# AndreasKarg/raytracer-weekend

Measured on AMD Instinct MI355X. Metric: Mrays/sec at 1920x1080, 512 spp, 50 bounces; 1/2/4/8-GPU scaling, higher is better.
Workload: dtype f32; 1 GPU; Random-spheres scene, 1920x1080, 512 spp, 1xMI355X (configs[1]); scene=jumpy-balls, width=1920, height=1080, spp=512, max_depth=50, rays_per_frame=3103484398, tiles=32400, launches_per_frame=1, parallelism=tiles1

## Files before the change

raytracer-weekend_amd/csrc/rtw_dev_trace.hpp:

```cpp
#pragma once
#include "rtw_dev_hit.hpp"

namespace rtw {
namespace dev {

struct TraceState {
  Best b;
  int32_t node;
  int32_t pend;
  int32_t sp;
  bool on;
};

template <int AXIS, bool FAST>
__device__ __forceinline__ void rect_list_test(const Ray& lr, V3 y, float4 q0, float k, uint32_t pi, float& bt,
                                               int32_t& bp) {
  const float o_k = AXIS == 0 ? lr.o.z : (AXIS == 1 ? lr.o.y : lr.o.x);
  const float d_k = AXIS == 0 ? lr.d.z : (AXIS == 1 ? lr.d.y : lr.d.x);
  const float y_k = AXIS == 0 ? y.z : (AXIS == 1 ? y.y : y.x);
  const float o_a = AXIS == 2 ? lr.o.y : lr.o.x, d_a = AXIS == 2 ? lr.d.y : lr.d.x;
  const float o_b = AXIS == 0 ? lr.o.y : lr.o.z, d_b = AXIS == 0 ? lr.d.y : lr.d.z;
  const float num = k - o_k;
  bool acc;
  if constexpr (FAST) {
    const float t = div_by_recip(num, d_k, y_k);
    const float x = o_a + t * d_a;
    const float yy = o_b + t * d_b;
    const float m1 = __builtin_amdgcn_fmed3f(t, TMIN, bt), m2 = __builtin_amdgcn_fmed3f(x, q0.x, q0.y);
    const float m3 = __builtin_amdgcn_fmed3f(yy, q0.z, q0.w);
    acc = fmaxf(fmaxf(fabsf(m1 - t), fabsf(m2 - x)), fabsf(m3 - yy)) == 0.0f;
    bt = acc ? t : bt;
    bp = acc ? (int32_t)pi : bp;
  } else {
    const float t = num / d_k;
    const float x = o_a + t * d_a;
    const float yy = o_b + t * d_b;
    const bool out = (x < q0.x) | (x > q0.y) | (yy < q0.z) | (yy > q0.w);
    acc = !(t < TMIN) & !(t > bt) & !out;
    const bool tnan = t != t;
    bt = acc ? (tnan ? INFINITY : t) : bt;
    bp = acc ? ((int32_t)pi | (tnan ? RECT_NAN_HIT : 0)) : bp;
  }
}

template <bool COUNT, int AXIS, bool FAST>
__device__ __forceinline__ void rect_list_run(const DevScene& S, uint32_t first, uint32_t count, const Ray& lr, V3 y,
                                              float& bt, int32_t& bp, uint32_t* cnt) {
  typedef uint32_t u8v __attribute__((ext_vector_type(8)));
  const __attribute__((address_space(4))) u8v* P = (const __attribute__((address_space(4))) u8v*)(S.prims + first);
  auto one = [&](const u8v& rec, uint32_t k) {
    const float4 q0 = make_float4(__uint_as_float(rec[0]), __uint_as_float(rec[1]), __uint_as_float(rec[2]),
                                  __uint_as_float(rec[3]));
    rect_list_test<AXIS, FAST>(lr, y, q0, __uint_as_float(rec[4]), first + k, bt, bp);
    if (COUNT) { cnt[1]++; cnt[2 + PT_RECT_XY + AXIS]++; simd_tick(cnt, 10, 11); }
  };
  uint32_t k = 0;
  const __attribute__((address_space(4))) u8v* Pk = P;
  for (; k + 1u < count; k += 2u, Pk += 4) {
    const u8v r0 = Pk[0], r1 = Pk[2];
    one(r0, k);
    one(r1, k + 1u);
  }
  if (k < count) {
    const u8v rl = Pk[0];
    one(rl, k);
  }
}

template <bool COUNT, bool FAST>
__device__ __forceinline__ void rect_box6_run(const DevScene& S, uint32_t first, const Ray& lr, V3 y, float& bt,
                                              int32_t& bp, uint32_t* cnt) {
  rect_list_run<COUNT, 0, FAST>(S, first, 2u, lr, y, bt, bp, cnt);
  rect_list_run<COUNT, 1, FAST>(S, first + 2u, 2u, lr, y, bt, bp, cnt);
  rect_list_run<COUNT, 2, FAST>(S, first + 4u, 2u, lr, y, bt, bp, cnt);
}

template <bool COUNT>
__device__ __forceinline__ void trace_rect_list(const DevScene& S, const Ray& r, Best& best, uint32_t* cnt) {
  float bt = INFINITY;
  int32_t bp = -1;
  uint32_t cur = 0xFFFFFFFFu;
  Ray lr = r;
  V3 y = mk(0.f, 0.f, 0.f);
  bool fast = false;
  for (uint32_t g = 0; g < S.n_lgroups; ++g) {
    const uint4 G = uload(reinterpret_cast<const uint4*>(S.lgroups + g));
    if (G.z != cur) {
      cur = G.z;
      lr = r;
      if (cur) {
        const DevInst* I = S.insts + cur;
        const uint32_t n = uload(&I->nops);
        const float4 op0 = uload(reinterpret_cast<const float4*>(I->op[0]));
        const float4 op1 = uload(reinterpret_cast<const float4*>(I->op[1]));
        auto apply = [&](const float4& op) {
          if (op_is(op.x, IO_TRANSLATE)) {
            lr.o = sub(lr.o, mk(op.y, op.z, op.w));
          } else {
            const float sn = op.y, c = op.z;
            lr.o = mk(c * lr.o.x - sn * lr.o.z, lr.o.y, sn * lr.o.x + c * lr.o.z);
            lr.d = mk(c * lr.d.x - sn * lr.d.z, lr.d.y, sn * lr.d.x + c * lr.d.z);
          }
        };
        if (n >= 1u) apply(op0);
        if (n >= 2u) apply(op1);
        for (uint32_t k = 2; k < n; ++k) apply(uload(reinterpret_cast<const float4*>(I->op[k])));
      }
      y = mk(rcp_rn_fast(lr.d.x), rcp_rn_fast(lr.d.y), rcp_rn_fast(lr.d.z));
      const float dmin = fminf(fminf(fabsf(lr.d.x), fabsf(lr.d.y)), fabsf(lr.d.z));
      const float dsum = (fabsf(lr.d.x) + fabsf(lr.d.y)) + fabsf(lr.d.z);
      const float osum = (fabsf(lr.o.x) + fabsf(lr.o.y)) + fabsf(lr.o.z);
      const bool ok = (dmin >= 0x1p-60f) & (dsum <= 0x1p60f) & (osum < 0x1p62f);
      fast = S.rect_fast && __ballot(!ok) == 0;
    }
    if (fast) {
      if (G.w == GK_BOX6) rect_box6_run<COUNT, true>(S, G.x, lr, y, bt, bp, cnt);
      else if (G.w == PT_RECT_XY) rect_list_run<COUNT, 0, true>(S, G.x, G.y, lr, y, bt, bp, cnt);
      else if (G.w == PT_RECT_XZ) rect_list_run<COUNT, 1, true>(S, G.x, G.y, lr, y, bt, bp, cnt);
      else rect_list_run<COUNT, 2, true>(S, G.x, G.y, lr, y, bt, bp, cnt);
    } else {
      if (G.w == GK_BOX6) rect_box6_run<COUNT, false>(S, G.x, lr, y, bt, bp, cnt);
      else if (G.w == PT_RECT_XY) rect_list_run<COUNT, 0, false>(S, G.x, G.y, lr, y, bt, bp, cnt);
      else if (G.w == PT_RECT_XZ) rect_list_run<COUNT, 1, false>(S, G.x, G.y, lr, y, bt, bp, cnt);
      else rect_list_run<COUNT, 2, false>(S, G.x, G.y, lr, y, bt, bp, cnt);
    }
  }
  const bool nan_hit = bp >= 0 && (bp & RECT_NAN_HIT) != 0;
  best.t = nan_hit ? __builtin_nanf("") : bt;
  best.prim = nan_hit ? (bp & ~RECT_NAN_HIT) : bp;
}

__device__ __forceinline__ const DevFar* far_record(const DevScene& S) {
  const char* p = reinterpret_cast<const char*>(S.prims);
  asm volatile("" : "+s"(p));
  return reinterpret_cast<const DevFar*>(p - DEVFAR_BACK);
}
__device__ __forceinline__ float cull_inv(float d) {
  const float dd = fabsf(d) > 1e-20f ? d : copysignf(1e-20f, d);
  return __builtin_amdgcn_rcpf(dd);
}
__device__ __forceinline__ float cull_tmax(float t) { return __builtin_fmaf(t, 1.0e-5f, t) + 1.0e-5f; }
template <bool COUNT, uint32_t FEAT, int STACK, int BLK, bool C16, int NCAP>
__device__ void trace_far(const DevScene& S, const Ray& r, Best& b, float delta, uint16_t* stk16, int32_t* stk,
                          uint32_t* cnt, uint64_t seg, uint32_t* err, const float4* lnodes) {
  const DevFar* const FR = far_record(S);
  const char* const NB = NCAP > 0 ? reinterpret_cast<const char*>(lnodes)
                                  : reinterpret_cast<const char*>(S.prims) - uload(&FR->nodes_back);
  const uint32_t n_bvh = uload(&FR->n_bvh);
  const V3 inv = mk(cull_inv(r.d.x), cull_inv(r.d.y), cull_inv(r.d.z));
  const V3 ood = mk(r.o.x * inv.x, r.o.y * inv.y, r.o.z * inv.z);
  const V3 bn = mk(-ood.x - delta * fabsf(inv.x), -ood.y - delta * fabsf(inv.y), -ood.z - delta * fabsf(inv.z));
  const V3 bf = mk(-ood.x + delta * fabsf(inv.x), -ood.y + delta * fabsf(inv.y), -ood.z + delta * fabsf(inv.z));
  const uint32_t nx = inv.x < 0.f ? 16u : 0u, ny = (inv.y < 0.f ? 16u : 0u) + 32u, nz = (inv.z < 0.f ? 16u : 0u) + 64u;
  const uint32_t fx = nx ^ 16u, fy = ny ^ 16u, fz = nz ^ 16u;
  int32_t node = 0, sp = 0;
  bool over = false;
  for (uint32_t guard = 0;; ++guard) {
    if (node < 0) {
      if (sp == 0) break;
      --sp;
      node = C16 ? (int32_t)stk16[sp * BLK] : stk[sp * BLK];
    }
    if (guard >= (1u << 20)) {
      *err = 1u;
      b.prim = -2;
      return;
    }
    if (COUNT) cnt[0]++;
    const uint32_t nb = (uint32_t)node << 7;
    const float4 qnx = *reinterpret_cast<const float4*>(NB + (nb + nx)), qfx = *reinterpret_cast<const float4*>(NB + (nb + fx));
    const float4 qny = *reinterpret_cast<const float4*>(NB + (nb + ny)), qfy = *reinterpret_cast<const float4*>(NB + (nb + fy));
    const float4 qnz = *reinterpret_cast<const float4*>(NB + (nb + nz)), qfz = *reinterpret_cast<const float4*>(NB + (nb + fz));
    const uint4 cw = *reinterpret_cast<const uint4*>(NB + (nb + (C16 ? 112u : 96u)));
    const float tmax_c = cull_tmax(b.t);
    const float NX[4] = {qnx.x, qnx.y, qnx.z, qnx.w}, FX[4] = {qfx.x, qfx.y, qfx.z, qfx.w};
    const float NY[4] = {qny.x, qny.y, qny.z, qny.w}, FY[4] = {qfy.x, qfy.y, qfy.z, qfy.w};
    const float NZ[4] = {qnz.x, qnz.y, qnz.z, qnz.w}, FZ[4] = {qfz.x, qfz.y, qfz.z, qfz.w};
    const uint32_t W[4] = {cw.x, cw.y, cw.z, cw.w};
    uint32_t hits = 0;
    float tnear = INFINITY;
    int kn = -1;
#pragma unroll
    for (int k = 0; k < 4; ++k) {
      const float tn = fmaxf(fmaxf(fmaxf(__builtin_fmaf(NX[k], inv.x, bn.x), __builtin_fmaf(NY[k], inv.y, bn.y)),
                                   __builtin_fmaf(NZ[k], inv.z, bn.z)), 0.0f);
      const float tf = fminf(fminf(fminf(__builtin_fmaf(FX[k], inv.x, bf.x), __builtin_fmaf(FY[k], inv.y, bf.y)),
                                   __builtin_fmaf(FZ[k], inv.z, bf.z)), tmax_c);
      const bool h = W[k] != 0u && tn <= tf;
      hits |= h ? 1u << k : 0u;
      const bool inner = C16 ? (W[k] & 0x8000u) == 0u : (int32_t)W[k] >= 0;
      const bool nearer = h && inner && tn < tnear;
      tnear = nearer ? tn : tnear;
      kn = nearer ? k : kn;
    }
    node = kn < 0 ? -1 : (int32_t)(kn == 0 ? W[0] : (kn == 1 ? W[1] : (kn == 2 ? W[2] : W[3])));
    hits &= kn < 0 ? hits : ~(1u << kn);
    while (hits) {
      const int k = __builtin_ctz(hits);
      hits &= hits - 1u;
      const uint32_t w = k == 0 ? W[0] : (k == 1 ? W[1] : (k == 2 ? W[2] : W[3]));
      if (C16 ? (w & 0x8000u) != 0u : (int32_t)w < 0) {
        const uint32_t v = C16 ? w & 0xFFFFu : ~w;
        const uint32_t first = C16 ? (v >> 2) & 0x1FFFu : v >> 3, n = C16 ? (v & 3u) + 1u : v & 7u;
        for (uint32_t q = 0; q < n; ++q) test_prim<COUNT, FEAT>(S, first + q, r, b, cnt, seg);
      } else if (sp < STACK) {
        if constexpr (C16) stk16[sp * BLK] = (uint16_t)w;
        else stk[sp * BLK] = (int32_t)w;
        ++sp;
      } else {
        over = true;
      }
    }
  }
  if (over)
    for (uint32_t pi = 0; pi < n_bvh; ++pi) test_prim<COUNT, FEAT>(S, pi, r, b, cnt, seg);
}

constexpr bool far_kernel_feat(uint32_t feat) {
  return !(feat & F_LIST) && (feat & (F_SPHERE | F_MSPHERE | F_MEDIUM)) && feat != F_MESHES;
}
template <bool COUNT, uint32_t FEAT, int STACK = 1, int BLK = BLOCK, bool C16 = false, int NCAP = 0, bool RING = false>
__device__ __forceinline__ void trace_begin(const DevScene& S, const Ray& r, TraceState& ts, uint32_t* cnt,
                                            uint64_t seg, uint16_t* stk16 = nullptr, int32_t* stk = nullptr,
                                            uint32_t* err = nullptr, const float4* lnodes = nullptr,
                                            int32_t start = -3) {
  ts.b = Best{INFINITY, 0u, -1, 0.0f, 0.0f};
  const bool decided = RING && start != -3;
  constexpr bool RECT_LIST = (FEAT & F_LIST) && (FEAT & F_RECT) && !(FEAT & (F_SPHERE | F_MSPHERE | F_TRI | F_MEDIUM));
  if constexpr (RECT_LIST) {
    trace_rect_list<COUNT>(S, r, ts.b, cnt);
  } else if (FEAT & F_INST) {
    uint32_t cur = 0;
    Ray lr = r;
    const uint32_t a0 = S.n_prims - S.n_always;
    for (uint32_t k = 0; k < S.n_always; ++k) {
      const uint32_t pi = a0 + k;
      const uint32_t inst = uload(&S.prims[pi].type_inst) >> 8;
      if (inst != cur) {
        lr = inst ? to_local<true>(S.insts + inst, r) : r;
        cur = inst;
      }
      test_prim<COUNT, FEAT, true, true>(S, pi, lr, ts.b, cnt, seg);
    }
  } else if constexpr (RING) {
    const SphRcp rq = sph_rcp(r);
    const uint32_t n = decided ? (start >= 0 ? 1u : 0u) : S.n_always;
    for (uint32_t k = 0; __any(k < n); ++k) {
      if (k < n) {
        const uint32_t pi = decided ? (uint32_t)start : uload(S.always + k);
        test_prim<COUNT, FEAT, false, false>(S, pi, r, ts.b, cnt, seg, &rq);
      }
    }
  } else {
    constexpr bool SPH_ONLY = (FEAT & (F_RECT | F_TRI | F_MEDIUM | F_INST)) == 0 && (FEAT & (F_SPHERE | F_MSPHERE));
    SphRcp rq;
    if constexpr (SPH_ONLY) rq = sph_rcp(r);
    for (uint32_t k = 0; k < S.n_always; ++k)
      test_prim<COUNT, FEAT, false, true>(S, uload(S.always + k), r, ts.b, cnt, seg, SPH_ONLY ? &rq : nullptr);
  }
  if constexpr ((FEAT & F_LIST) && !RECT_LIST) {
    const bool nan_hit = ts.b.prim >= 0 && (ts.b.prim & RECT_NAN_HIT) != 0;
    ts.b.t = nan_hit ? __builtin_nanf("") : ts.b.t;
    ts.b.prim = nan_hit ? (ts.b.prim & ~RECT_NAN_HIT) : ts.b.prim;
  }
  bool walk = true;
#if defined(RTW_DIAG_FAR)
  constexpr int DF = RTW_DIAG_FAR;
#else
  constexpr int DF = 0;
#endif
  constexpr bool FAR = DF != 1 && far_kernel_feat(FEAT);
  if constexpr (FAR) {
    if (S.far_check) {
      const float4* const FR = reinterpret_cast<const float4*>(far_record(S));
      const float4 mid = uload(FR), half = uload(FR + 1);
      const float tx = fabsf(r.o.x - mid.x) + half.x;
      const float ty = fabsf(r.o.y - mid.y) + half.y;
      const float tz = fabsf(r.o.z - mid.z) + half.z;
      const float D2 = tx * tx + ty * ty + tz * tz;
      const bool far = D2 > mid.w && !decided;
      if (__any(far)) {
        bool need = false;
        float delta = 0.0f;
        if (far && DF != 2) {
          const float4 lo = uload(FR + 2), hi = uload(FR + 3), e = uload(FR + 4);
          const float D = __builtin_amdgcn_sqrtf(D2) * 1.000001f;
          delta = fminf(half.w * D2 + lo.w, hi.w * D + e.x) + (e.y * D + e.z);
          const float ix = __builtin_amdgcn_rcpf(r.d.x), iy = __builtin_amdgcn_rcpf(r.d.y), iz = __builtin_amdgcn_rcpf(r.d.z);
          const float ox = r.o.x - mid.x, oy = r.o.y - mid.y, oz = r.o.z - mid.z;
          const float hx = half.x + delta, hy = half.y + delta, hz = half.z + delta;
          const float ax = (-hx - ox) * ix, bx = (hx - ox) * ix, ay = (-hy - oy) * iy, by = (hy - oy) * iy;
          const float az = (-hz - oz) * iz, bz = (hz - oz) * iz;
          const float tn = fmaxf(fmaxf(fminf(ax, bx), fminf(ay, by)), fmaxf(fminf(az, bz), 0.0f));
          const float tf = fminf(fminf(fmaxf(ax, bx), fmaxf(ay, by)),
                                 fminf(fmaxf(az, bz), cull_tmax(ts.b.t)));
          need = tn <= tf;
        }
        walk = !far;
        if (DF == 5) asm volatile("" ::"v"((uint32_t)need));
        if (DF != 3 && DF != 5 && __builtin_expect(__any(need), 0))
          if (need) trace_far<COUNT, FEAT, STACK, BLK, C16, NCAP>(S, r, ts.b, delta, stk16, stk, cnt, seg, err, lnodes);
      }
    }
  }
  int32_t root = S.n_nodes ? 0 : -1;
  if constexpr ((FEAT & F_TRI) != 0) {
    root = __builtin_amdgcn_readfirstlane(root);
    asm volatile("" : "+s"(root));
  } else {
    asm volatile("" : "+v"(root));
  }
  ts.node = (walk && !decided) ? root : -1;
  ts.pend = 0;
  ts.sp = 0;
  ts.on = true;
}

#ifndef RTW_MESH_ROOT
#define RTW_MESH_ROOT 5
#endif
#ifndef REGEN_RING
#define REGEN_RING 2
#endif
#ifndef REGEN_RING_LDSN
#define REGEN_RING_LDSN 8
#endif
typedef _Float16 half2_t __attribute__((ext_vector_type(2)));
__device__ __forceinline__ half2_t as_h2(uint32_t u) { return __builtin_bit_cast(half2_t, u); }

template <bool COUNT, int STACK, bool SPILL, uint32_t FEAT, int BLK, int NCAP, bool HN = false, bool S16 = false>
__device__ void trace_run(const DevScene& S, const Ray& r, TraceState& ts, int32_t* stk, int32_t* spill,
                          uint32_t spill_lanes, uint32_t* cnt, uint32_t quota, uint32_t leaf_thr, uint64_t seg,
                          uint32_t* err, uint64_t* tph, const float4* lnodes, uint16_t* stk16) {
  constexpr bool K16 = NCAP > 0;
  constexpr bool CODES = K16 || HN || S16;
  constexpr bool SPH_ONLY = (FEAT & (F_RECT | F_TRI | F_MEDIUM | F_INST)) == 0 && (FEAT & (F_SPHERE | F_MSPHERE));
  SphRcp rq;
  if constexpr (SPH_ONLY) rq = sph_rcp(r);
  Ray tri_ray = r;
  if constexpr ((FEAT & F_TRI) != 0) {
    if (S.bvh_tri && (FEAT & F_INST) && S.tri_inst) {
      if (S.tri_inst == S.uni_inst) tri_ray.o = sub(r.o, mk(S.uni_off[0], S.uni_off[1], S.uni_off[2]));
      else tri_ray = to_local<true>(S.insts + S.tri_inst, r);
    }
  }
  uint64_t tm = COUNT ? __builtin_amdgcn_s_memtime() : 0;
  if constexpr (NCAP == 0) __builtin_amdgcn_s_setprio(2);
  auto tick = [&](int k) {
    if (COUNT) {
      const uint64_t t = __builtin_amdgcn_s_memtime();
      tph[k] += t - tm;
      tm = t;
    }
  };
  const V3 inv = mk(cull_inv(r.d.x), cull_inv(r.d.y), cull_inv(r.d.z));
  const V3 ood = mk(r.o.x * inv.x, r.o.y * inv.y, r.o.z * inv.z);
  const uint32_t nx = inv.x < 0.f ? 16u : 0u, ny = (inv.y < 0.f ? 16u : 0u) + 32u, nz = (inv.z < 0.f ? 16u : 0u) + 64u;
  const uint32_t fx = nx ^ 16u, fy = ny ^ 16u, fz = nz ^ 16u;
  const char* const NB = NCAP > 0 ? reinterpret_cast<const char*>(lnodes)
                                  : (HN ? reinterpret_cast<const char*>(S.hnodes) : reinterpret_cast<const char*>(S.nodes));
  constexpr bool ROOT = HN && S16 && NCAP == 0 && RTW_MESH_ROOT > 0;
  constexpr int32_t NROOT = RTW_MESH_ROOT;
#pragma unroll
  for (int lv = 0; lv < (ROOT ? (NROOT > 1 ? 2 : 1) : 0); ++lv) {
    if (__any(ts.node >= 0 && ts.node < NROOT)) {
      if (ts.node >= 0 && ts.node < NROOT) {
        const char* const TB = reinterpret_cast<const char*>(lnodes) + (uint32_t)ts.node * 112u;
        const uint4 px = *reinterpret_cast<const uint4*>(TB + nx);
        const uint4 py = *reinterpret_cast<const uint4*>(TB + ny);
        const uint4 pz = *reinterpret_cast<const uint4*>(TB + nz);
        const uint4 cq = *reinterpret_cast<const uint4*>(TB + 96u);
        const half2_t oxy = as_h2(cq.z), oz = as_h2(cq.w);
        const V3 bs = mk(__builtin_fmaf((float)oxy.x, inv.x, -ood.x), __builtin_fmaf((float)oxy.y, inv.y, -ood.y),
                         __builtin_fmaf((float)oz.x, inv.z, -ood.z));
        const uint32_t PQ[3][4] = {{px.x, px.y, px.z, px.w}, {py.x, py.y, py.z, py.w}, {pz.x, pz.y, pz.z, pz.w}};
        float NA[3][4], FA[3][4];
#pragma unroll
        for (int q = 0; q < 3; ++q) {
          const half2_t n01 = as_h2(PQ[q][0]), n23 = as_h2(PQ[q][1]), f01 = as_h2(PQ[q][2]), f23 = as_h2(PQ[q][3]);
          NA[q][0] = (float)n01.x; NA[q][1] = (float)n01.y; NA[q][2] = (float)n23.x; NA[q][3] = (float)n23.y;
          FA[q][0] = (float)f01.x; FA[q][1] = (float)f01.y; FA[q][2] = (float)f23.x; FA[q][3] = (float)f23.y;
        }
        const int32_t CW[4] = {(int32_t)(int16_t)(cq.x & 0xFFFFu), (int32_t)cq.x >> 16, (int32_t)(int16_t)(cq.y & 0xFFFFu),
                               (int32_t)cq.y >> 16};
        if (COUNT) {
          cnt[0]++;
          cnt[14] += (CW[0] != 0) + (CW[1] != 0) + (CW[2] != 0) + (CW[3] != 0);
        }
        const float tmax_c = cull_tmax(ts.b.t);
        int32_t next = -1, bk = -1;
        float best = INFINITY;
        bool hit[4];
#pragma unroll
        for (int k = 0; k < 4; ++k) {
          const float a0 = __builtin_fmaf(NA[0][k], inv.x, bs.x), b0 = __builtin_fmaf(NA[1][k], inv.y, bs.y);
          const float c0 = __builtin_fmaf(NA[2][k], inv.z, bs.z);
          const float d0 = __builtin_fmaf(FA[0][k], inv.x, bs.x), e0 = __builtin_fmaf(FA[1][k], inv.y, bs.y);
          const float f0 = __builtin_fmaf(FA[2][k], inv.z, bs.z);
          const float tn = fmaxf(fmaxf(fmaxf(a0, b0), c0), 0.0f);
          hit[k] = tn <= fminf(fminf(fminf(d0, e0), f0), tmax_c);
          const bool in = hit[k] & (CW[k] >= 0) & (tn < best);
          best = in ? tn : best;
          bk = in ? k : bk;
          next = in ? CW[k] : next;
        }
        int32_t pend = ts.pend, sp = ts.sp;
#pragma unroll
        for (int k = 0; k < 4; ++k) {
          const bool leaf_take = hit[k] & (CW[k] < 0) & (pend == 0);
          pend = leaf_take ? CW[k] : pend;
          const bool pk = hit[k] & (k != bk) & !leaf_take;
          stk16[sp * BLK] = (uint16_t)CW[k];
          sp += pk ? 1 : 0;
        }
        ts.pend = pend;
        ts.sp = sp;
        ts.node = next;
      }
    }
  }
  constexpr uint32_t GUARD = 1u << 20;
  uint32_t guard = 0;
  for (; guard < GUARD; ++guard) {
    uint32_t g2 = 0;
    for (; g2 < GUARD; ++g2) {
      if constexpr (K16) {
        const bool can = ts.node < 0 && ts.sp > 0;
        const int32_t top = can ? (int32_t)stk16[(ts.sp - 1) * BLK] : 0;
        const bool leaf = (top & 0x8000) != 0;
        const bool popn = can && !leaf;
        const bool popl = can && leaf && ts.pend == 0;
        ts.node = popn ? top : ts.node;
        ts.pend = popl ? top : ts.pend;
        ts.sp -= (popn || popl) ? 1 : 0;
      } else {
        const bool can = ts.node < 0 && ts.sp > 0;
        int32_t top = 0;
        if (can) {
          const int32_t i = ts.sp - 1;
          if constexpr (S16) {
            top = (int32_t)(int16_t)stk16[i * BLK];
          } else {
            top = stk[(SPILL ? min(i, STACK) : i) * BLK];
            if (SPILL && i >= STACK) top = spill[(size_t)(i - STACK) * spill_lanes];
          }
        }
        const bool popn = can && top >= 0;
        const bool popl = can && top < 0 && ts.pend == 0;
        ts.node = popn ? top : ts.node;
        ts.pend = popl ? top : ts.pend;
        ts.sp -= (popn || popl) ? 1 : 0;
      }
#ifdef RTW_LANE_DIAG
      if (COUNT) {
        const uint64_t bd = __ballot(ts.node >= 0), bp = __ballot(ts.node < 0 && ts.pend != 0);
        const uint64_t bn = __ballot(ts.node < 0 && ts.pend == 0 && ts.sp == 0);
        tph[3] += 64;
        tph[4] += (uint64_t)__popcll(bd);
        tph[5] += (uint64_t)__popcll(bp);
        tph[6] += (uint64_t)__popcll(bn);
      }
#endif
      if (!__any(ts.node >= 0 && ts.pend == 0)) break;
      if ((uint32_t)__popcll(__ballot(ts.node < 0 && ts.pend != 0)) >= leaf_thr) break;
#ifdef RTW_UNI_DIAG
      if (COUNT) {
        const uint64_t vis = __ballot(ts.node >= 0);
        const int src = (int)__ffsll((long long)vis) - 1;
        const int32_t n0 = __shfl(ts.node, src, 64);
        const uint32_t oct = nx | ny | nz, o0 = (uint32_t)__shfl((int)oct, src, 64);
        const bool un = __ballot(ts.node >= 0 && ts.node != n0) == 0;
        const bool uo = __ballot(ts.node >= 0 && (ts.node != n0 || oct != o0)) == 0;
        tph[3] += 1;
        tph[4] += uo ? 1 : 0;
        tph[5] += un ? 1 : 0;
        tph[6] += (uint64_t)__popcll(vis);
      }
#endif
      if (ts.node >= 0) {
        float NX[4], FX[4], NY[4], FY[4], NZ[4], FZ[4];
        int32_t CW[4];
        V3 bs;
        if constexpr (HN) {
          const uint32_t nb = (uint32_t)ts.node * 112u;
          const uint4 px = *reinterpret_cast<const uint4*>(NB + (nb + nx));
          const uint4 py = *reinterpret_cast<const uint4*>(NB + (nb + ny));
          const uint4 pz = *reinterpret_cast<const uint4*>(NB + (nb + nz));
          const uint4 cq = *reinterpret_cast<const uint4*>(NB + (nb + 96u));
          const half2_t oxy = as_h2(cq.z), oz = as_h2(cq.w);
          bs = mk(__builtin_fmaf((float)oxy.x, inv.x, -ood.x), __builtin_fmaf((float)oxy.y, inv.y, -ood.y),
                  __builtin_fmaf((float)oz.x, inv.z, -ood.z));
          const uint32_t P[3][4] = {{px.x, px.y, px.z, px.w}, {py.x, py.y, py.z, py.w}, {pz.x, pz.y, pz.z, pz.w}};
          float* const NA[3] = {NX, NY, NZ};
          float* const FA[3] = {FX, FY, FZ};
#pragma unroll
          for (int a = 0; a < 3; ++a) {
            const half2_t n01 = as_h2(P[a][0]), n23 = as_h2(P[a][1]), f01 = as_h2(P[a][2]), f23 = as_h2(P[a][3]);
            NA[a][0] = (float)n01.x; NA[a][1] = (float)n01.y; NA[a][2] = (float)n23.x; NA[a][3] = (float)n23.y;
            FA[a][0] = (float)f01.x; FA[a][1] = (float)f01.y; FA[a][2] = (float)f23.x; FA[a][3] = (float)f23.y;
          }
          if constexpr (K16) {
            CW[0] = (int32_t)(cq.x & 0xFFFFu); CW[1] = (int32_t)(cq.x >> 16);
            CW[2] = (int32_t)(cq.y & 0xFFFFu); CW[3] = (int32_t)(cq.y >> 16);
          } else {
            CW[0] = (int32_t)(int16_t)(cq.x & 0xFFFFu); CW[1] = (int32_t)cq.x >> 16;
            CW[2] = (int32_t)(int16_t)(cq.y & 0xFFFFu); CW[3] = (int32_t)cq.y >> 16;
          }
        } else {
          const uint32_t nb = (uint32_t)ts.node << 7;
          constexpr uint32_t CWO = (K16 || S16) ? 112u : 96u;
          const float4 qnx = *reinterpret_cast<const float4*>(NB + (nb + nx));
          const float4 qfx = *reinterpret_cast<const float4*>(NB + (nb + fx));
          const float4 qny = *reinterpret_cast<const float4*>(NB + (nb + ny));
          const float4 qfy = *reinterpret_cast<const float4*>(NB + (nb + fy));
          const float4 qnz = *reinterpret_cast<const float4*>(NB + (nb + nz));
          const float4 qfz = *reinterpret_cast<const float4*>(NB + (nb + fz));
          const int4 cw = *reinterpret_cast<const int4*>(NB + (nb + CWO));
          bs = neg(ood);
          NX[0] = qnx.x; NX[1] = qnx.y; NX[2] = qnx.z; NX[3] = qnx.w; FX[0] = qfx.x; FX[1] = qfx.y; FX[2] = qfx.z; FX[3] = qfx.w;
          NY[0] = qny.x; NY[1] = qny.y; NY[2] = qny.z; NY[3] = qny.w; FY[0] = qfy.x; FY[1] = qfy.y; FY[2] = qfy.z; FY[3] = qfy.w;
          NZ[0] = qnz.x; NZ[1] = qnz.y; NZ[2] = qnz.z; NZ[3] = qnz.w; FZ[0] = qfz.x; FZ[1] = qfz.y; FZ[2] = qfz.z; FZ[3] = qfz.w;
          if constexpr (S16 && !K16) {
            CW[0] = (int32_t)(int16_t)cw.x; CW[1] = (int32_t)(int16_t)cw.y;
            CW[2] = (int32_t)(int16_t)cw.z; CW[3] = (int32_t)(int16_t)cw.w;
          } else {
            CW[0] = cw.x; CW[1] = cw.y; CW[2] = cw.z; CW[3] = cw.w;
          }
        }
        if (COUNT) {
          cnt[0]++;
          simd_tick(cnt, 8, 9);
          cnt[14] += (CW[0] != 0) + (CW[1] != 0) + (CW[2] != 0) + (CW[3] != 0);
        }
        const float tmax_c = cull_tmax(ts.b.t);
        float tn[4];
        bool hit[4];
#pragma unroll
        for (int k = 0; k < 4; ++k) {
          const float a = __builtin_fmaf(NX[k], inv.x, bs.x), b = __builtin_fmaf(NY[k], inv.y, bs.y);
          const float c = __builtin_fmaf(NZ[k], inv.z, bs.z);
          const float d = __builtin_fmaf(FX[k], inv.x, bs.x), e = __builtin_fmaf(FY[k], inv.y, bs.y);
          const float f = __builtin_fmaf(FZ[k], inv.z, bs.z);
          tn[k] = fmaxf(fmaxf(fmaxf(a, b), c), 0.0f);
          hit[k] = tn[k] <= fminf(fminf(fminf(d, e), f), tmax_c);
        }
        if constexpr (K16) {
          int32_t cwv[4] = {CW[0], CW[1], CW[2], CW[3]};
          asm volatile("" : "+v"(cwv[0]), "+v"(cwv[1]), "+v"(cwv[2]), "+v"(cwv[3]));
          uint32_t key[4];
// ... 84 lines not shown
```

raytracer-weekend_amd/csrc/rtw_path_kernel.hpp:

```cpp
#pragma once
#include "rtw_dev_shade.hpp"
#include "rtw_dev_trace.hpp"

namespace rtw {
namespace dev {

constexpr uint32_t BATCH = 2048;

struct PathState {
  Ray ray;
  V3 T;
  uint64_t rng;
  uint32_t pid;
  uint32_t depth;
};

__device__ __forceinline__ uint32_t fastdiv(uint32_t n, uint64_t M) {
  const uint64_t t = (uint64_t)(uint32_t)(M >> 32) * n + __umulhi((uint32_t)M, n);
  return (uint32_t)(t >> 32);
}

__device__ __forceinline__ uint64_t rfl64(uint64_t x) {
  const uint32_t hi = (uint32_t)__builtin_amdgcn_readfirstlane((int)(uint32_t)(x >> 32));
  const uint32_t lo = (uint32_t)__builtin_amdgcn_readfirstlane((int)(uint32_t)x);
  return ((uint64_t)hi << 32) | lo;
}

struct StartArgs {
  DevCamera cam;
  float fw1, fh1, rw1, rh1, time_span;
  uint32_t w, h, spp, max_depth, tiles_x, slot_base, tile_first, tile_stride;
  uint64_t spp_magic, tiles_x_magic, seed_hash;
  const uint32_t* tile_ids;
};
__device__ __forceinline__ void fill_start_args(const RenderArgs& a, StartArgs& o) {
  o.cam = a.cam;
  o.fw1 = a.fw1; o.fh1 = a.fh1; o.rw1 = a.rw1; o.rh1 = a.rh1; o.time_span = a.time_span;
  o.w = a.w; o.h = a.h; o.spp = a.spp; o.max_depth = a.max_depth; o.tiles_x = a.tiles_x;
  o.slot_base = a.slot_base; o.tile_first = a.tile_first; o.tile_stride = a.tile_stride;
  o.spp_magic = a.spp_magic; o.tiles_x_magic = a.tiles_x_magic; o.seed_hash = a.seed_hash;
  o.tile_ids = a.tile_ids;
}

struct StartMade {
  float rdx, rdy;
  float u, v;
  V3 d;
  uint64_t rng;
  uint32_t tile;
};
constexpr int32_t START_MISS = -1, START_WALK = -3;
template <bool FROM_LDS, bool AB>
__device__ __forceinline__ bool start_make(const StartArgs& a, uint64_t pid, StartMade& m) {
  if constexpr (FROM_LDS) asm volatile("" ::: "memory");
  const uint32_t hi = (uint32_t)(pid >> 6), l = (uint32_t)pid & 63u;
  const uint32_t slot = a.spp > 1u ? fastdiv(hi, a.spp_magic) : hi, s = hi - slot * a.spp;
  const uint32_t gslot = a.slot_base + slot;
  const uint32_t tile = a.tile_ids ? a.tile_ids[gslot] : a.tile_first + gslot * a.tile_stride;
  const uint32_t ty = a.tiles_x > 1u ? fastdiv(tile, a.tiles_x_magic) : tile;
  const uint32_t i = (tile - ty * a.tiles_x) * 8u + (l & 7u), row = ty * 8u + (l >> 3);
  const uint32_t j = a.h - 1u - row;
  const DevCamera& C = a.cam;
  uint64_t rng = xoro_seed(splitmix64(a.seed_hash ^ (((uint64_t)j << 48) | ((uint64_t)i << 32) | s)));
  const float u = div_by_recip((float)i + gen_f32(rng), a.fw1, a.rw1);
  const float v = div_by_recip((float)j + gen_f32(rng), a.fh1, a.rh1);
  const V3 rd = scale(rand_in_unit_disk<AB>(rng), C.lens_radius);
  const V3 off = add(scale(ld3(C.u), rd.x), scale(ld3(C.v), rd.y));
  m.rdx = rd.x;
  m.rdy = rd.y;
  m.u = u;
  m.v = v;
  m.tile = tile;
  m.d = sub(sub(add(add(ld3(C.llc), scale(ld3(C.horizontal), u)), scale(ld3(C.vertical), v)), ld3(C.origin)), off);
  m.rng = rng;
  return i < a.w && row < a.h;
}
template <bool FENCE, bool AB>
__device__ __forceinline__ void start_take(const StartArgs& a, float rdx, float rdy, float u, float v, uint64_t rng,
                                           uint32_t pid, PathState& st) {
  if constexpr (FENCE) asm volatile("" ::: "memory");
  const DevCamera& C = a.cam;
  const V3 off = add(scale(ld3(C.u), rdx), scale(ld3(C.v), rdy));
  st.ray.o = add(ld3(C.origin), off);
  st.ray.d = sub(sub(add(add(ld3(C.llc), scale(ld3(C.horizontal), u)), scale(ld3(C.vertical), v)), ld3(C.origin)), off);
  st.ray.time = gen_range<AB>(rng, C.time0, C.time1, a.time_span);
  st.rng = rng;
  st.T = mk(1.f, 1.f, 1.f);
  st.depth = a.max_depth;
  st.pid = pid;
}

template <bool COUNT, uint32_t FEAT, bool AB>
__device__ __forceinline__ int32_t start_decide(const DevScene& S, const StartArgs& a, const uint32_t* lists,
                                                const StartMade& m, uint32_t* cnt) {
  if (!lists) return START_WALK;
  const uint32_t tile = (uint32_t)__builtin_amdgcn_readfirstlane((int)m.tile);
  if (tile >= a.tiles_x * ((a.h + 7u) >> 3)) return START_WALK;
  const uint32_t* const rec = lists + (size_t)tile * TILE_LIST_WORDS;
  const uint32_t w0 = uload(rec);
  const uint32_t n = w0 & 0xFFFFu;
  if (n == TILE_LIST_OVER) return START_WALK;
  const DevCamera& C = a.cam;
  Ray r;
  const V3 off = add(scale(ld3(C.u), m.rdx), scale(ld3(C.v), m.rdy));
  r.o = add(ld3(C.origin), off);
  r.d = m.d;
  uint64_t g = m.rng;
  r.time = gen_range<AB>(g, C.time0, C.time1, a.time_span);
  const SphRcp rq = sph_rcp(r);
  Best b = Best{INFINITY, 0u, -1, 0.0f, 0.0f};
  for (uint32_t k = 0; k < S.n_always; ++k) test_prim<COUNT, FEAT, false, true>(S, uload(S.always + k), r, b, cnt, g, &rq);
  for (uint32_t k = 1; k <= n; ++k) {
    const uint32_t pi = (uload(rec + (k >> 1)) >> ((k & 1u) * 16u)) & 0xFFFFu;
    test_prim<COUNT, FEAT, false, true>(S, pi, r, b, cnt, g, &rq);
  }
  return b.prim;
}

template <bool FROM_LDS, int LST_BLK = 0, int LST_ROW = 0, bool AB = FROM_LDS>
__device__ __forceinline__ bool start_path(const StartArgs& a, uint64_t pid, PathState& st, uint16_t* lst = nullptr) {
  if constexpr (FROM_LDS) asm volatile("" ::: "memory");
  const uint32_t hi = (uint32_t)(pid >> 6), l = (uint32_t)pid & 63u;
  const uint32_t slot = a.spp > 1u ? fastdiv(hi, a.spp_magic) : hi, s = hi - slot * a.spp;
  const uint32_t gslot = a.slot_base + slot;
  const uint32_t tile = a.tile_ids ? a.tile_ids[gslot] : a.tile_first + gslot * a.tile_stride;
  const uint32_t ty = a.tiles_x > 1u ? fastdiv(tile, a.tiles_x_magic) : tile;
  const uint32_t i = (tile - ty * a.tiles_x) * 8u + (l & 7u), row = ty * 8u + (l >> 3);
  if (i >= a.w || row >= a.h) return false;
  const uint32_t j = a.h - 1u - row;
  const DevCamera& C = a.cam;
  uint64_t rng = xoro_seed(splitmix64(a.seed_hash ^ (((uint64_t)j << 48) | ((uint64_t)i << 32) | s)));
  const float u = div_by_recip((float)i + gen_f32(rng), a.fw1, a.rw1);
  const float v = div_by_recip((float)j + gen_f32(rng), a.fh1, a.rh1);
  const V3 rd = scale(rand_in_unit_disk<AB>(rng), C.lens_radius);
  const V3 off = add(scale(ld3(C.u), rd.x), scale(ld3(C.v), rd.y));
  st.ray.o = add(ld3(C.origin), off);
  st.ray.d = sub(sub(add(add(ld3(C.llc), scale(ld3(C.horizontal), u)), scale(ld3(C.vertical), v)), ld3(C.origin)),
                 off);
  st.ray.time = gen_range<AB>(rng, C.time0, C.time1, a.time_span);
  st.rng = rng;
  st.T = mk(1.f, 1.f, 1.f);
  st.depth = a.max_depth;
  st.pid = (uint32_t)pid;
  if constexpr (LST_BLK > 0) {
    const uint32_t v[5] = {0x3F800000u, 0x3F800000u, 0x3F800000u, a.max_depth, (uint32_t)pid};
#pragma unroll
    for (int k = 0; k < 5; ++k) {
      lst[(LST_ROW + 2 * k) * LST_BLK] = (uint16_t)v[k];
      lst[(LST_ROW + 2 * k + 1) * LST_BLK] = (uint16_t)(v[k] >> 16);
    }
  }
  return true;
}

struct KernelCfg {
  int stack;
  bool spill;
  int occ;
  uint32_t feat;
  int blk = BLOCK;
  int ncap = 0;
  bool half = false;
  bool s16 = false;
  constexpr bool lds_nodes() const { return ncap > 0; }
  constexpr bool ldsn_ring() const { return ncap > 0 && blk == 1024 && feat == F_SPHERES; }
  constexpr int lst_rows() const { return s16 ? 10 : 0; }
  constexpr int lst_row0() const { return stack + (s16 ? 1 : 0); }
  constexpr bool lst() const { return lst_rows() > 0; }
  constexpr bool shard() const { return ncap > 0; }
  constexpr bool sring() const { return feat == (F_BOXES | F_LIST) || ldsn_ring(); }
  constexpr int ring_words() const { return ldsn_ring() ? 7 : 10; }
  constexpr bool root_lds() const { return half && s16 && ncap == 0 && RTW_MESH_ROOT > 0; }
  constexpr bool alignbit_draws() const { return !(feat & F_TRI); }
  constexpr bool start_args_in_lds() const { return alignbit_draws() || s16; }
  constexpr uint32_t node_quads() const { return half ? 7u : 8u; }
  constexpr bool codes16_stack() const { return ncap > 0 || s16; }
  constexpr int far_lds_nodes() const { return half ? 0 : ncap; }
  constexpr int stk_words() const { return codes16_stack() ? 1 : (stack + 1) * blk; }
  constexpr int stk16_words(int more = 0) const { return ncap > 0 ? stack * blk : (s16 ? (stack + 1 + more) * blk : 1); }
  constexpr uint32_t lds_node_quads() const {
    return ncap > 0 ? ncap * node_quads() : (root_lds() ? RTW_MESH_ROOT * node_quads() : 1u);
  }
};

template <KernelCfg K>
__device__ __forceinline__ void fill_nodes_lds(const DevScene& S, float4* nodes_lds) {
  if constexpr (K.ncap > 0) {
    const float4* g = K.half ? reinterpret_cast<const float4*>(S.hnodes) : reinterpret_cast<const float4*>(S.nodes);
    for (uint32_t k = threadIdx.x; k < S.n_nodes * K.node_quads(); k += K.blk) nodes_lds[k] = g[k];
  }
  if constexpr (K.root_lds()) {
    const uint32_t nq = min(S.n_nodes, (uint32_t)RTW_MESH_ROOT) * K.node_quads();
    if (threadIdx.x < nq) nodes_lds[threadIdx.x] = reinterpret_cast<const float4*>(S.hnodes)[threadIdx.x];
  }
}

template <bool COUNT, KernelCfg K>
__global__ __launch_bounds__(K.blk) __attribute__((amdgpu_waves_per_eu(K.occ, 8))) void path_kernel(RenderArgs a) {
  __shared__ int32_t stk_all[K.stk_words()];
  __shared__ uint16_t stk16_all[K.stk16_words(K.lst_rows())];
  __shared__ float4 nodes_lds[K.lds_node_quads()];
  fill_nodes_lds<K>(a.scene, nodes_lds);
  __shared__ StartArgs start_lds[K.start_args_in_lds() ? 1 : 0 + 1];
  StartArgs sa_reg;
  if constexpr (K.start_args_in_lds()) {
    if (threadIdx.x == 0) fill_start_args(a, start_lds[0]);
  } else {
    fill_start_args(a, sa_reg);
  }
  const StartArgs& SA = K.start_args_in_lds() ? start_lds[0] : sa_reg;
  __syncthreads();
  uint16_t* stk16 = stk16_all + threadIdx.x;
  int32_t* stk = stk_all + threadIdx.x;
  int32_t* spill = a.spill + (size_t)blockIdx.x * K.blk + threadIdx.x;
  const uint32_t lane = threadIdx.x & 63u;
  constexpr bool LST = K.lst();
  auto lst_st = [&](int k, uint32_t v) {
    stk16[(K.lst_row0() + 2 * k) * K.blk] = (uint16_t)v;
    stk16[(K.lst_row0() + 2 * k + 1) * K.blk] = (uint16_t)(v >> 16);
  };
  auto lst_ld = [&](int k) -> uint32_t {
    return (uint32_t)stk16[(K.lst_row0() + 2 * k) * K.blk] | ((uint32_t)stk16[(K.lst_row0() + 2 * k + 1) * K.blk] << 16);
  };
  const DevScene& S = a.scene;
  const V3 bg = ld3(a.bg);
  const uint64_t P = a.n_paths;
  unsigned long long* const dispenser = a.queue;
  const uint32_t batch = a.batch, ndisp = batch < 1024u ? DISP : 1u;
  const uint64_t NB = (P + batch - 1u) / batch;
  uint32_t cnt[15] = {0, 0, 0, 0, 0, 0, 0, 0, 0, 0, 0, 0, 0, 0, 0};
  unsigned long long nrays = 0;
  __shared__ uint64_t pool_lds[K.blk / 64][K.shard() ? 5 : 3];
  uint64_t* const pool = pool_lds[K.s16 ? __builtin_amdgcn_readfirstlane(threadIdx.x >> 6) : threadIdx.x >> 6];
  if (lane == 0) { pool[0] = 0; pool[1] = 0; }
  if (K.shard() && lane == 0) pool[K.shard() ? 4 : 0] = 0;
  auto refill = [&](uint64_t& b, uint64_t& e) {
    if (lane == 0) {
      uint64_t bb = P, ee = P;
      uint32_t k = (uint32_t)pool[4];
      for (; k < ndisp; ++k) {
        const uint32_t d = (blockIdx.x + k) & (ndisp - 1u);
        const uint64_t g = atomicAdd(dispenser + d * DISP_STRIDE, 1ull) * ndisp + d;
        if (g < NB) {
          bb = g * batch;
          ee = bb + batch < P ? bb + batch : P;
          break;
        }
      }
      pool[2] = bb;
      pool[K.shard() ? 3 : 0] = ee;
      pool[K.shard() ? 4 : 0] = k;
    }
    b = rfl64(pool[2]);
    e = rfl64(pool[K.shard() ? 3 : 0]);
  };
  constexpr uint32_t RW = K.ring_words(), RS = RW * 64u + (K.ldsn_ring() ? 2u : 0u);
  __shared__ uint32_t ring_lds[K.sring() ? (K.blk / 64) * RS : 1];
  __shared__ uint32_t ring_head_lds[K.sring() && !K.ldsn_ring() ? K.blk / 64 : 1];
  if constexpr (K.ldsn_ring()) {
    static_assert(sizeof stk_all + sizeof stk16_all + sizeof nodes_lds + sizeof start_lds + sizeof pool_lds +
                          sizeof ring_lds + sizeof ring_head_lds <= 81920,
                  "the 1024-lane ring kernel's LDS must leave room for 2 workgroups per CU");
  }
  uint32_t* const ring = ring_lds + (K.sring() ? (threadIdx.x >> 6) * RS : 0u);
  uint32_t* const ring_head = K.ldsn_ring() ? ring + RW * 64u : ring_head_lds + (K.sring() ? threadIdx.x >> 6 : 0u);
  uint32_t* const ring_base = ring + (K.ldsn_ring() ? RW * 64u + 1u : 0u);
  if (K.sring() && lane == 0) ring_head[0] = 64u;
  bool exhausted = false;
  bool has = false;
  int32_t start_win = START_WALK;
  TraceState ts;
  ts.on = false;
  PathState st;
  st.pid = 0;
  st.rng = 0;
  st.depth = 0;
  uint64_t ph[11] = {0, 0, 0, 0, 0, 0, 0, 0, 0, 0, 0};
  const uint64_t t_start = COUNT ? __builtin_amdgcn_s_memtime() : 0;
  uint64_t t_mark = t_start;
  auto phase = [&](int k) {
    if (COUNT) {
      const uint64_t t = __builtin_amdgcn_s_memtime();
      ph[k] += t - t_mark;
      t_mark = t;
    }
  };
  for (;;) {
    phase(2);
    const uint64_t need = __ballot(!has);
    if constexpr (K.sring()) {
      if (need != 0 && !exhausted && ((uint32_t)__popcll(need) >= a.regen_min || need == __ballot(1))) {
        const uint32_t n_need = (uint32_t)__popcll(need);
        const uint32_t rank =
            __builtin_amdgcn_mbcnt_hi((uint32_t)(need >> 32), __builtin_amdgcn_mbcnt_lo((uint32_t)need, 0u));
        const uint64_t t_sp = COUNT ? __builtin_amdgcn_s_memtime() : 0;
        uint32_t head = (uint32_t)__builtin_amdgcn_readfirstlane((int)ring_head[0]);
        const uint32_t have = 64u - head;
        auto take = [&](uint32_t e) {
          if constexpr (K.ldsn_ring()) {
            const uint32_t lo = ring[5 * 64 + e], hi = ring[6 * 64 + e];
            const float rdx = __uint_as_float(ring[e]), rdy = __uint_as_float(ring[64 + e]);
            start_take<true, K.alignbit_draws()>(SA, rdx, rdy, __uint_as_float(ring[2 * 64 + e]),
                                                 __uint_as_float(ring[3 * 64 + e]), ((uint64_t)hi << 32) | lo,
                                                 ring_base[0] + e, st);
            start_win = (int32_t)ring[4 * 64 + e];
            has = (lo | hi) != 0u;
          } else {
            const uint32_t lo = ring[7 * 64 + e], hi = ring[8 * 64 + e];
            st.ray.o = mk(__uint_as_float(ring[e]), __uint_as_float(ring[64 + e]), __uint_as_float(ring[2 * 64 + e]));
            st.ray.d = mk(__uint_as_float(ring[3 * 64 + e]), __uint_as_float(ring[4 * 64 + e]),
                          __uint_as_float(ring[5 * 64 + e]));
            st.ray.time = __uint_as_float(ring[6 * 64 + e]);
            st.rng = ((uint64_t)hi << 32) | lo;
            st.pid = ring[9 * 64 + e];
            st.T = mk(1.f, 1.f, 1.f);
            st.depth = SA.max_depth;
            has = (lo | hi) != 0u;
          }
        };
        const bool first = !has && rank < have;
        if (first) take(head + rank);
        if (n_need > have) {
          uint64_t pool_next = rfl64(pool[0]), pool_end = rfl64(pool[1]);
          if (pool_next >= pool_end) {
            if constexpr (K.shard()) {
              refill(pool_next, pool_end);
            } else {
              if (lane == 0) pool[2] = atomicAdd(dispenser, (unsigned long long)batch);
              const uint64_t b = rfl64(pool[2]);
              pool_next = b < P ? b : P;
              pool_end = b < P ? (b + batch < P ? b + batch : P) : P;
            }
          }
          if (pool_next < pool_end) {
            const uint64_t id = pool_next + lane;
            if constexpr (K.ldsn_ring()) {
              StartMade m;
              const bool ok = start_make<K.start_args_in_lds(), K.alignbit_draws()>(SA, id, m);
              const int32_t win = start_decide<COUNT, K.feat, K.alignbit_draws()>(S, SA, a.tile_lists, m, cnt);
              ring[lane] = __float_as_uint(m.rdx);
              ring[64 + lane] = __float_as_uint(m.rdy);
              ring[2 * 64 + lane] = __float_as_uint(m.u);
              ring[3 * 64 + lane] = __float_as_uint(m.v);
              ring[4 * 64 + lane] = (uint32_t)win;
              ring[5 * 64 + lane] = ok ? (uint32_t)m.rng : 0u;
              ring[6 * 64 + lane] = ok ? (uint32_t)(m.rng >> 32) : 0u;
              if (lane == 0) ring_base[0] = (uint32_t)pool_next;
            } else {
              PathState g;
              const bool ok = start_path<K.start_args_in_lds(), 0, 0, K.alignbit_draws()>(SA, id, g);
              ring[lane] = __float_as_uint(g.ray.o.x);
              ring[64 + lane] = __float_as_uint(g.ray.o.y);
              ring[2 * 64 + lane] = __float_as_uint(g.ray.o.z);
              ring[3 * 64 + lane] = __float_as_uint(g.ray.d.x);
              ring[4 * 64 + lane] = __float_as_uint(g.ray.d.y);
              ring[5 * 64 + lane] = __float_as_uint(g.ray.d.z);
              ring[6 * 64 + lane] = __float_as_uint(g.ray.time);
              ring[7 * 64 + lane] = ok ? (uint32_t)g.rng : 0u;
              ring[8 * 64 + lane] = ok ? (uint32_t)(g.rng >> 32) : 0u;
              ring[9 * 64 + lane] = (uint32_t)id;
            }
            pool_next += 64u;
            if (!has && !first) take(rank - have);
            head = n_need - have;
          } else {
            exhausted = true;
            head = 64u;
          }
          if (lane == 0) { pool[0] = pool_next; pool[1] = pool_end; }
        } else {
          head += n_need;
        }
        if (lane == 0) ring_head[0] = head;
        if (COUNT) ph[6] += __builtin_amdgcn_s_memtime() - t_sp;
      }
    } else if (need != 0 && !exhausted && ((uint32_t)__popcll(need) >= a.regen_min || need == __ballot(1))) {
      const uint32_t n_need = (uint32_t)__popcll(need);
      const uint32_t rank =
          __builtin_amdgcn_mbcnt_hi((uint32_t)(need >> 32), __builtin_amdgcn_mbcnt_lo((uint32_t)need, 0u));
      uint64_t pool_next = rfl64(pool[0]), pool_end = rfl64(pool[1]);
      const uint64_t avail = pool_end - pool_next;
      uint64_t nb = P, ne = P;
      if (avail < n_need) {
        if constexpr (K.shard()) {
          uint64_t b, e;
          refill(b, e);
          if (b < e) {
            nb = b;
            ne = e;
          } else {
            exhausted = true;
          }
        } else {
          if (lane == 0) pool[2] = atomicAdd(dispenser, (unsigned long long)batch);
          const uint64_t b = rfl64(pool[2]);
          if (b < P) {
            nb = b;
            ne = b + batch < P ? b + batch : P;
          } else {
            exhausted = true;
          }
        }
      }
      const uint64_t t_sp = COUNT ? __builtin_amdgcn_s_memtime() : 0;
      if (!has) {
        const uint64_t id = rank < avail ? pool_next + rank : nb + (rank - avail);
        if ((rank < avail || id < ne) &&
            start_path<K.start_args_in_lds(), LST ? K.blk : 0, K.lst_row0(), K.alignbit_draws()>(SA, id, st, stk16)) {
          has = true;
        }
      }
      if (COUNT) ph[6] += __builtin_amdgcn_s_memtime() - t_sp;
      if (avail >= n_need) {
        pool_next += n_need;
      } else {
        pool_next = nb + (n_need - avail);
        pool_end = ne;
        if (pool_next > pool_end) pool_next = pool_end;
      }
      if (lane == 0) { pool[0] = pool_next; pool[1] = pool_end; }
    }
    phase(0);
    if (__ballot(has) == 0) {
      if (exhausted) break;
      continue;
    }
    nrays += (unsigned long long)__popcll(__ballot(has && !ts.on));
    if (!has) continue;
    bool decided = false;
    if (!ts.on) {
      if constexpr (K.ldsn_ring()) {
        decided = start_win != START_WALK;
        trace_begin<COUNT, K.feat, K.stack, K.blk, K.codes16_stack(), K.far_lds_nodes(), true>(
            S, st.ray, ts, cnt, st.rng, stk16, stk, a.err, nodes_lds, start_win);
        start_win = START_WALK;
      } else {
        trace_begin<COUNT, K.feat, K.stack, K.blk, K.codes16_stack(), K.far_lds_nodes()>(S, st.ray, ts, cnt, st.rng, stk16,
                                                                                         stk, a.err, nodes_lds);
      }
    }
    if (!(K.feat & F_LIST)) {
      const uint32_t act = (uint32_t)__popcll(__ballot(1));
      const uint32_t ndec = K.ldsn_ring() ? (uint32_t)__popcll(__ballot(decided)) : 0u;
      const uint32_t quota = (((act - ndec) * a.quota16 + 15u) >> 4) + ndec;
      const uint32_t leaf_thr = (act * a.leaf16 + 15u) >> 4;
      trace_run<COUNT, K.stack, K.spill, K.feat, K.blk, K.ncap, K.half, K.s16>(S, st.ray, ts, stk, spill, a.spill_lanes, cnt,
                                                                              quota, leaf_thr, st.rng, a.err, ph + 4, nodes_lds, stk16);
    } else {
      ts.node = -1;
      ts.sp = 0;
    }
    phase(1);
    __builtin_amdgcn_s_setprio(0);
    if (ts.node >= 0 || ts.sp > 0) continue;
    ts.on = false;
    if (COUNT) simd_tick(cnt, 12, 13);
    const Best b = ts.b;
#ifdef RTW_DIAG_TRACE_PID
    if ((RTW_DIAG_TRACE_PID) < 0 || st.pid == (uint32_t)(RTW_DIAG_TRACE_PID))
      printf("rtwtrace pid %u o %a %a %a d %a %a %a t %a prim %d key %u rng %016llx\n", st.pid, st.ray.o.x, st.ray.o.y,
             st.ray.o.z, st.ray.d.x, st.ray.d.y, st.ray.d.z, b.t, b.prim, b.prim >= 0 ? S.prims[b.prim].key : 0u,
             (unsigned long long)st.rng);
#endif
    bool done = false;
    V3 L = mk(0.f, 0.f, 0.f);
    const V3 T0 = st.T;
    auto path_T = [&]() -> V3 {
      return LST ? mk(__uint_as_float(lst_ld(0)), __uint_as_float(lst_ld(1)), __uint_as_float(lst_ld(2))) : T0;
    };
    if (b.prim < 0) {
      L = mul(path_T(), bg);
      done = true;
      if (__builtin_expect(b.prim == -2, 0)) {
        if constexpr (K.shard()) {
          for (uint32_t d = 0; d < DISP; ++d) atomicMax(dispenser + d * DISP_STRIDE, (unsigned long long)NB);
        } else {
          atomicMax(dispenser, (unsigned long long)P);
        }
        pool[0] = pool[1];
        if constexpr (K.ldsn_ring()) ring_head[0] = 64u;
      }
    } else {
      DevShade sh;
      if constexpr (LST) {
        const float4 q = *reinterpret_cast<const float4*>(S.shade + b.prim);
        sh.kind = __float_as_uint(q.x); sh.param = q.y; sh.a[0] = q.z; sh.a[1] = q.w;
        sh.a[2] = S.shade[b.prim].a[2];
      } else {
        sh = S.shade[b.prim];
      }
      const bool solid_light = (K.feat & F_LIGHT) && (K.feat & F_TRI) && (sh.kind & 0xfffu) == (MT_LIGHT | (SM_SOLID << 8));
      Rec h;
      if (!solid_light) h = hit_record<K.feat>(S, st.ray, b, sh.kind);
      else h = Rec{mk(0.f, 0.f, 0.f), mk(0.f, 0.f, 0.f), 0.0f, 0.0f, true, 0u};
#ifdef RTW_SHADE_DIAG
      phase(7);
#endif
      const MatKind kind = mat_kind<K.feat>(sh.kind);
      V3 rs = mk(0.f, 0.f, 0.f);
      phase(2);
      if (kind.lam || kind.met || kind.iso) rs = rand_in_unit_sphere<K.alignbit_draws()>(st.rng);
      phase(3);
      const V3 ud = unit(kind.lam ? rs : st.ray.d);
      const V3 att = mat_attenuation<K.feat>(S, sh, kind, h, [&] { return ld3(LST ? S.shade[b.prim].b : sh.b); });
#ifdef RTW_SHADE_DIAG
      phase(8);
#endif
      V3 Tn = mk(0.f, 0.f, 0.f);
      if (kind.light) {
        L = mul(path_T(), att);
        done = true;
      } else {
        const V3 dir = mat_direction<K.feat>(sh, kind, h, ud, rs, st.rng, done);
        const V3 Tp = path_T();
        const V3 T2 = mul(Tp, att);
        if (done) L = mul(Tp, mk(0.f, 0.f, 0.f));
        Tn = T2;
        if constexpr (LST) {
          lst_st(0, __float_as_uint(T2.x));
          lst_st(1, __float_as_uint(T2.y));
          lst_st(2, __float_as_uint(T2.z));
        } else {
          st.T = T2;
        }
        st.ray.o = h.p;
        st.ray.d = dir;
      }
#ifdef RTW_SHADE_DIAG
      phase(9);
#endif
      if (!done) {
        if constexpr (LST) {
          const uint32_t d = lst_ld(3) - 1u;
          lst_st(3, d);
          done = d == 0u;
        } else {
          done = --st.depth == 0u;
        }
        if (done) L = mul(Tn, mk(0.f, 0.f, 0.f));
      }
    }
    if (done) {
      float* o = a.sbuf + (size_t)(LST ? lst_ld(4) : st.pid) * 3u;
#ifdef RTW_DIAG_NO_STORE
      if (L.x == -1.2345f) o[0] = L.y;
#else
#if RTW_NT_SAMPLES
      __builtin_nontemporal_store(L.x, o);
      __builtin_nontemporal_store(L.y, o + 1);
      __builtin_nontemporal_store(L.z, o + 2);
#else
      o[0] = L.x;
      o[1] = L.y;
      o[2] = L.z;
#endif
#endif
      has = false;
    }
  }
  if (lane == 0 && nrays) atomicAdd(a.counters, nrays);
  if (COUNT) {
    phase(2);
    if (lane == 0) {
      for (int k = 0; k < 3; ++k) atomicAdd(a.counters + 16 + k, (unsigned long long)ph[k]);
      atomicAdd(a.counters + 19, (unsigned long long)(t_mark - t_start));
#if defined(RTW_LANE_DIAG) || defined(RTW_UNI_DIAG) || defined(RTW_SHADE_DIAG)
      for (int k = 7; k < 11; ++k) atomicAdd(a.counters + 13 + k, (unsigned long long)ph[k]);
#else
      for (int k = 3; k < 7; ++k) atomicAdd(a.counters + 17 + k, (unsigned long long)ph[k]);
#endif
    }
    for (int q = 0; q < 15; ++q) {
      unsigned long long c = cnt[q];
      for (int off = 32; off > 0; off >>= 1) c += __shfl_xor(c, off, 64);
      if (lane == 0 && c) atomicAdd(a.counters + 1 + q, c);
    }
  }
}

}
}
```

Baseline: 28780 Mrays/s.

## Resolve sky-miss camera rays at generation and compact live starts in ring

```diff
diff --git a/raytracer-weekend_amd/csrc/rtw_dev_trace.hpp b/raytracer-weekend_amd/csrc/rtw_dev_trace.hpp
--- a/raytracer-weekend_amd/csrc/rtw_dev_trace.hpp
+++ b/raytracer-weekend_amd/csrc/rtw_dev_trace.hpp
@@ -244,7 +244,7 @@
     }
   } else if constexpr (RING) {
     const SphRcp rq = sph_rcp(r);
-    const uint32_t n = decided ? (start >= 0 ? 1u : 0u) : S.n_always;
+    const uint32_t n = decided ? 1u : S.n_always;
     for (uint32_t k = 0; __any(k < n); ++k) {
       if (k < n) {
         const uint32_t pi = decided ? (uint32_t)start : uload(S.always + k);
diff --git a/raytracer-weekend_amd/csrc/rtw_path_kernel.hpp b/raytracer-weekend_amd/csrc/rtw_path_kernel.hpp
--- a/raytracer-weekend_amd/csrc/rtw_path_kernel.hpp
+++ b/raytracer-weekend_amd/csrc/rtw_path_kernel.hpp
@@ -50,6 +50,7 @@
   uint32_t tile;
 };
 constexpr int32_t START_MISS = -1, START_WALK = -3;
+constexpr uint32_t RING_WALK = 0xFFFFu;
 template <bool FROM_LDS, bool AB>
 __device__ __forceinline__ bool start_make(const StartArgs& a, uint64_t pid, StartMade& m) {
   if constexpr (FROM_LDS) asm volatile("" ::: "memory");
@@ -300,11 +301,12 @@
           if constexpr (K.ldsn_ring()) {
             const uint32_t lo = ring[5 * 64 + e], hi = ring[6 * 64 + e];
             const float rdx = __uint_as_float(ring[e]), rdy = __uint_as_float(ring[64 + e]);
+            const uint32_t ww = ring[4 * 64 + e];
             start_take<true, K.alignbit_draws()>(SA, rdx, rdy, __uint_as_float(ring[2 * 64 + e]),
                                                  __uint_as_float(ring[3 * 64 + e]), ((uint64_t)hi << 32) | lo,
-                                                 ring_base[0] + e, st);
-            start_win = (int32_t)ring[4 * 64 + e];
-            has = (lo | hi) != 0u;
+                                                 ring_base[0] + (ww >> 16), st);
+            start_win = (ww & 0xFFFFu) == RING_WALK ? START_WALK : (int32_t)(ww & 0xFFFFu);
+            has = true;
           } else {
             const uint32_t lo = ring[7 * 64 + e], hi = ring[8 * 64 + e];
             st.ray.o = mk(__uint_as_float(ring[e]), __uint_as_float(ring[64 + e]), __uint_as_float(ring[2 * 64 + e]));
@@ -334,17 +336,40 @@
           }
           if (pool_next < pool_end) {
             const uint64_t id = pool_next + lane;
+            [[maybe_unused]] uint32_t n_made = 64u;
             if constexpr (K.ldsn_ring()) {
               StartMade m;
               const bool ok = start_make<K.start_args_in_lds(), K.alignbit_draws()>(SA, id, m);
               const int32_t win = start_decide<COUNT, K.feat, K.alignbit_draws()>(S, SA, a.tile_lists, m, cnt);
-              ring[lane] = __float_as_uint(m.rdx);
-              ring[64 + lane] = __float_as_uint(m.rdy);
-              ring[2 * 64 + lane] = __float_as_uint(m.u);
-              ring[3 * 64 + lane] = __float_as_uint(m.v);
-              ring[4 * 64 + lane] = (uint32_t)win;
-              ring[5 * 64 + lane] = ok ? (uint32_t)m.rng : 0u;
-              ring[6 * 64 + lane] = ok ? (uint32_t)(m.rng >> 32) : 0u;
+              const bool sky = ok && win == START_MISS;
+              if (sky) {
+                const V3 L = mul(mk(1.f, 1.f, 1.f), bg);
+                float* o = a.sbuf + (size_t)(uint32_t)id * 3u;
+#if RTW_NT_SAMPLES
+                __builtin_nontemporal_store(L.x, o);
+                __builtin_nontemporal_store(L.y, o + 1);
+                __builtin_nontemporal_store(L.z, o + 2);
+#else
+                o[0] = L.x;
+                o[1] = L.y;
+                o[2] = L.z;
+#endif
+              }
+              nrays += (unsigned long long)__popcll(__ballot(sky));
+              const bool live = ok && !sky;
+              const uint64_t lv = __ballot(live);
+              n_made = (uint32_t)__popcll(lv);
+              const uint32_t e = 64u - n_made +
+                                 __builtin_amdgcn_mbcnt_hi((uint32_t)(lv >> 32), __builtin_amdgcn_mbcnt_lo((uint32_t)lv, 0u));
+              if (live) {
+                ring[e] = __float_as_uint(m.rdx);
+                ring[64 + e] = __float_as_uint(m.rdy);
+                ring[2 * 64 + e] = __float_as_uint(m.u);
+                ring[3 * 64 + e] = __float_as_uint(m.v);
+                ring[4 * 64 + e] = ((uint32_t)win < RING_WALK ? (uint32_t)win : RING_WALK) | (lane << 16);
+                ring[5 * 64 + e] = (uint32_t)m.rng;
+                ring[6 * 64 + e] = (uint32_t)(m.rng >> 32);
+              }
               if (lane == 0) ring_base[0] = (uint32_t)pool_next;
             } else {
               PathState g;
@@ -361,8 +386,14 @@
               ring[9 * 64 + lane] = (uint32_t)id;
             }
             pool_next += 64u;
-            if (!has && !first) take(rank - have);
-            head = n_need - have;
+            if constexpr (K.ldsn_ring()) {
+              const uint32_t head0 = 64u - n_made, want = n_need - have;
+              if (!has && !first && rank - have < n_made) take(head0 + (rank - have));
+              head = head0 + (want < n_made ? want : n_made);
+            } else {
+              if (!has && !first) take(rank - have);
+              head = n_need - have;
+            }
           } else {
             exhausted = true;
             head = 64u;
```

New measurement: 29170 Mrays/s, median of 6. +1.3%, better.
